# CG-Labs/HAN

Measured on AMD Instinct MI355X. Metric: full-graph train epochs/sec + node-attn HBM GB/s, 8-head HAN at 1/2/4/8 GPUs, higher is better.
Workload: dtype f32

## Files before the change

### han_amd/_lib.py

```python
from __future__ import annotations

import ctypes
import os
import subprocess
from ctypes import c_char_p, c_float, c_int, c_int64, c_size_t, c_uint64, c_void_p

_HERE = os.path.dirname(os.path.abspath(__file__))
LIB_PATH = os.path.join(_HERE, "libhan_hip.so")
CSRC = os.path.join(_HERE, "csrc")
SOURCES = ("node_attn.hip", "project.hip", "project_sparse.hip", "sem_attn.hip", "loss_opt.hip", "metapath.hip", "evaluate.hip",
           "ego_block.hip")
EXTRA_FLAGS = {"node_attn.hip": ("-mllvm", "-amdgpu-mfma-vgpr-form")}

P = c_void_p
I64 = c_int64


class HanRowSplit(ctypes.Structure):
    _fields_ = [("split_deg", c_int64), ("n_long", c_int64), ("n_chunks", c_int64),
                ("long_rows", c_void_p), ("long_ptr", c_void_p), ("chunk_long", c_void_p),
                ("chunk_start", c_void_p), ("chunk_end", c_void_p), ("workspace", c_void_p),
                ("workspace_bytes", c_size_t), ("n_short", c_int64), ("n_mid", c_int64),
                ("short_rows", c_void_p), ("mid_rows", c_void_p)]

# ... 1 lines not shown
class HanDense(ctypes.Structure):
    _fields_ = [("bits", c_void_p), ("ld_words", c_int64), ("n_table", c_int64), ("workspace", c_void_p),
                ("workspace_bytes", c_size_t)]


SIGNATURES = {
    "han_abi_version": (c_int, []),
    "han_error_string": (c_char_p, [c_int]),
    "han_project_fwd_workspace": (c_size_t, [I64, c_int, c_int, c_int]),
    "han_project_fwd_multi_workspace": (c_size_t, [I64, c_int, c_int, c_int, c_int]),
    "han_project_keep_bytes": (c_size_t, [I64, c_int, I64, c_int, c_int]),
    "han_project_fwd": (c_int, [P, c_int, I64, P, P, P, P, P, P, c_int, P, P, P, c_size_t, I64, c_int, c_int, c_int,
                                c_float, c_float, c_uint64, P, I64, P, c_int, P]),
    "han_project_fwd_multi": (c_int, [P, c_int, I64, P, P, P, P, P, P, c_int, P, P, P, c_size_t, I64, c_int, c_int, c_int,
                                      c_int, c_float, c_float, P, P, I64, P, c_int, P]),
    "han_project_bwd_workspace": (c_size_t, [I64, c_int, c_int, c_int]),
    "han_project_bwd": (c_int, [P, c_int, I64, P, P, P, c_size_t, I64, c_int, c_int, c_int, c_float,
                                c_uint64, P, I64, P, P]),
    "han_project_bwd_input": (c_int, [P, P, P, I64, I64, c_int, c_int, c_int, c_float, c_uint64, P, I64, P]),
    "han_project_sparse_fwd": (c_int, [P, P, P, P, P, P, P, P, P, c_int, P, P, I64, c_int, c_int, c_int, c_float, c_float,
                                       c_uint64, P, I64, c_int, P]),
    "han_project_sparse_bwd_workspace": (c_size_t, [I64]),
    "han_project_sparse_bwd": (c_int, [P, P, P, I64, I64, I64, P, P, P, P, P, P, P, P, c_size_t, I64, c_int, c_int, c_int,
                                       c_float, c_uint64, P, I64, P]),
    "han_row_split_workspace": (c_size_t, [I64]),
    "han_node_attn_fwd": (c_int, [P, P, P, P, c_int, P, P, P, P, P, P, P, P, I64, P, P, P, P, I64, I64, c_int,
                                  c_int, c_float, c_float, c_float, c_uint64, P, I64, c_int, c_int, P, P, P]),
    "han_node_attn_dense_workspace": (c_size_t, [I64, I64, c_int]),
    "han_csr_to_bitmask": (c_int, [P, P, I64, I64, P, I64, P, P]),
    "han_node_attn_coefs": (c_int, [P, P, P, P, P, P, P, c_int, I64, I64, c_int, c_int, c_float, c_float,
# ... 46 lines not shown
    "han_knn_topk": (c_int, [P, I64, P, I64, P, P, P, c_size_t, I64, I64, c_int, c_int, P]),
    "han_knn_vote": (c_int, [P, P, P, I64, c_int, I64, P]),
    "han_contingency": (c_int, [P, P, I64, c_int, c_int, P, P]),
    "han_kmeans_step_workspace": (c_size_t, [I64, c_int, c_int]),
    "han_kmeans_step": (c_int, [P, I64, P, P, P, P, P, P, P, P, P, c_size_t, I64, c_int, c_int, P]),
    "han_silhouette_workspace": (c_size_t, [I64, c_int, c_int]),
    "han_silhouette": (c_int, [P, I64, P, I64, c_int, c_int, P, P, P, P, P, c_size_t, P]),
    "han_tsne_workspace": (c_size_t, [I64, c_int]),
    "han_tsne_calibrate": (c_int, [P, I64, I64, c_int, c_float, c_float, c_int, c_int, P, P, P, P, P, P, c_size_t, P]),
    "han_tsne_step": (c_int, [P, I64, P, P, P, P, P, P, P, P, I64, c_int, c_float, c_float, c_float, c_float, c_int, P,
                              c_size_t, P]),
}

ABI_VERSION = 15
E_UNSUPPORTED = -2
_lib = None


class HanLibraryError(RuntimeError):
    pass


def build(force: bool = False, verbose: bool = False) -> str:
    from concurrent.futures import ThreadPoolExecutor
    hdrs = [os.path.join(CSRC, f) for f in os.listdir(CSRC) if f.endswith(".h")] + \
        [os.path.join(_HERE, "..", "include", "han_hip.h")]
    hdr_time = max(os.path.getmtime(h) for h in hdrs)
    objdir = os.path.join(CSRC, "build")
    os.makedirs(objdir, exist_ok=True)
    jobs, objs = [], []
# ... 59 lines not shown
```

### han_amd/csrc/loss_opt.hip

```cpp
#include "han_common.h"

namespace {

constexpr int MAXC = 16;
constexpr int kClsBlocks = 2048;

struct ClsArgs {
    const float *Z, *Wc, *bc;
    const int32_t *labels;
    const uint8_t *mask;
    float row_weight;
    float *logits, *dZ, *slab;
    int64_t N;
    int C, HC;
};

__device__ __forceinline__ float cls_row16_sum(float v) {
    v += han_dpp_xor16<1>(v);
    v += han_dpp_xor16<2>(v);
    v += han_dpp_xor16<4>(v);
    v += han_dpp_xor16<8>(v);
    return v;
}

// ... 462 lines not shown
    if (!bias || !rowptr || !colidx || N < 0 || ld < N) return HAN_E_BADARG;
    if (N == 0) return 0;
    bias_fill_kernel<<<(unsigned)((N + 3) / 4), 256, 0, (hipStream_t)stream>>>(bias, N, ld, rowptr, colidx);
    HAN_CHECK_LAUNCH();
    return 0;
}

extern "C" int han_abi_version(void) { return HAN_ABI_VERSION; }

extern "C" const char *han_error_string(int code) {
    switch (code) {
        case 0: return "ok";
        case HAN_E_BADARG: return "han: bad argument (null pointer, negative size or inconsistent shape)";
        case HAN_E_UNSUPPORTED: return "han: shape not supported by this build (K*FP == 64 with FP in {4,8,16,32,64}; D and A multiples of 64)";
        case HAN_E_WORKSPACE: return "han: workspace too small";
        default: return code > 0 ? hipGetErrorString((hipError_t)code) : "han: unknown error";
    }
}
```

### han_amd/csrc/project.hip

```cpp
#include "han_b6.h"
#include "han_k1_epilogue.h"

namespace {

constexpr int BM = 64;
constexpr int BK = 32;
constexpr int XS_LD = 34;
constexpr int WS_LD = 80;

struct ProjFwdArgs : K1Epilogue {
    const unsigned char *wimg;
    const void *X;
    int64_t ldx;
    const float *W;
    int x_bf16, F;
    uint32_t thr_in;
    float inv_keep_in;
    int f_chunk;
    float *partial;
    uint8_t *keep;
};

__device__ __forceinline__ float load_x1(const void *X, int bf, int64_t idx) {
    if (bf) return __uint_as_float((uint32_t)reinterpret_cast<const uint16_t *>(X)[idx] << 16);
// ... 340 lines not shown
#pragma unroll
    for (int m = 0; m < MT; ++m) {
#pragma unroll
        for (int r = 0; r < 4; ++r) {
            const int64_t row = row0 + 16 * (w * MT + m) + l4 * 4 + r;
            float vst[4];
#pragma unroll
            for (int t = 0; t < 4; ++t) {
                float v = acc[m][t][0][r];
                if (HPT > 1) v = myhh ? acc[m][t][HPT - 1][r] : v;
                if (DROP) v *= a.inv_keep_in;
                vst[t] = k1_store_elem(a, row, t, l15, v);
            }
            if (DROP && a.f1) tile_scores<8>(a, row, row < a.N, vst, a1c, a2c, l15);
        }
    }
}

struct ProjMultiArgs {
    const void *X;
    int64_t ldx;
    const float *W;
    const unsigned char *wimg;
    void *H;
    int h_bf16;
    int64_t N;
    int F;
    int p_first;
    int P;
    const float *a1, *a2, *b1, *b2;
// ... 722 lines not shown
        for (int p = 0; p < done && !m.fuse_scores; ++p) {
            rc = launch_scores(path_of(all, p, N, F, K, hb, kb), N, FP, h_bf16, st);
            if (rc != 0) return rc;
        }
    }
    for (int p = done; p < P; ++p) {
        const K1Path q = path_of(all, p, N, F, K, hb, kb);
        const int rc = han_project_fwd(X, x_dtype, ldx, q.W, q.a1, q.a2, q.b1, q.b2, q.H, table_dtype, q.f1, q.f2,
                                       workspace, workspace_bytes, N, F, K, FP, in_drop, fts_drop,
                                       seeds ? seeds[p] : 0, seed_dev, row_offset, q.keep, flags, stream);
        if (rc != 0) return rc;
    }
    return 0;
}

extern "C" size_t han_project_bwd_workspace(int64_t N, int F, int, int) {
    int ftiles; int64_t rpc, nch;
    bwd_geometry(N, F, &ftiles, &rpc, &nch);
    return (size_t)nch * (size_t)F * HAN_D * sizeof(float);
}

extern "C" int han_project_bwd(const void *X, int x_dtype, int64_t ldx, const float *dH, float *dW, void *workspace,
                               size_t workspace_bytes, int64_t N, int F, int K, int FP, float in_drop,
                               uint64_t seed, const uint64_t *seed_dev, int64_t row_offset, const uint8_t *keep,
                               void *stream) {
    if (!X || !dH || !dW || !workspace || N < 0 || F <= 0 || ldx < F) return HAN_E_BADARG;
    if (!han_fp_supported(K, FP)) return HAN_E_UNSUPPORTED;
    if (!han_k1_dtype(x_dtype)) return HAN_E_UNSUPPORTED;
    if (in_drop < 0.f || in_drop >= 1.f) return HAN_E_BADARG;
    if (workspace_bytes < han_project_bwd_workspace(N, F, K, FP)) return HAN_E_WORKSPACE;
// ... 44 lines not shown
```

### han_amd/gat.py

```python
from __future__ import annotations

import functools
import math

import torch
import torch.nn.functional as F_torch

from . import layers, ops, rng
from .base_gattn import BaseGAttN
from .dist import NodePartition
from .graph import CSRGraph, as_graph

D = ops.D


class _ClassOrInstance:

    def __init__(self, fn):
        self.fn = fn
        functools.update_wrapper(self, fn)

    def __get__(self, obj, objtype=None):
        if obj is None:
            obj = objtype.default_instance()
# ... 39 lines not shown
        torch.nn.Module.__init__(self)
        self._built = False
        self._device = torch.device(device) if device is not None else None
        self.partition: NodePartition | None = None
        self.halo_plans = (None, None)
        self.masked_bwd = None
        self.zero_rows = False
        self.live_bwd = None
        self.path_streams = None
        self.path_order = "index"
        self.overlap_branch = None
        self.fold_k3 = False
        self._fold_handover = None
        self._live_handover = None
        self.side_stream = None
        self._graph_cache: dict = {}
        self.step_seed_dev: torch.Tensor | None = None
        self._fixed_seeds: dict = {}

    @classmethod
    def default_instance(cls):
        if cls._default is None:
            cls._default = cls()
        return cls._default

    @classmethod
    def reset_default(cls):
        cls._default = None

    def build(self, n_metapaths, ft_size, nb_classes, hid_units=(8,), n_heads=(8, 1),
# ... 67 lines not shown
        if new_flat.dtype != torch.float32:
            raise TypeError("han_amd parameters are float32 (the kernels read fp32 parameters); "
                            "bf16 storage is selected with build(table_dtype=torch.bfloat16)")
        new_grad = fn(self.flat_grad)
        self._buffers["flat"], self._buffers["flat_grad"] = new_flat, new_grad
        off = 0
        for name, shp in self.param_shapes():
            n = math.prod(shp)
            v = self._views[name]
            v.data = new_flat[off:off + n].view(shp)
            v.grad = new_grad[off:off + n].view(shp)
            off += n
        self._graph_cache.clear()
        return self

    def param_shapes(self):
        return _param_shapes(self.P, self.F, self.K, self.FP, self.A, self.C, self.HC, self.extra,
                             self.residual)

    def direct_grads(self, flag: bool = True):
        for v in self._views.values():
            v._han_direct_grad = bool(flag)
        return self

    def zero_grad_flat(self):
        self.flat_grad.zero_()
        self._rebind_grads()

    def _rebind_grads(self):
        off = 0
# ... 39 lines not shown
            key = (layer, P)
            if key not in self._fixed_seeds:
                self._fixed_seeds[key] = tuple(rng.next_seed() for _ in graphs)
            return self._fixed_seeds[key]

        def run(layer, sd, **kw):
            first = layer == 0
            return layers.LayerRun(
                train=train, in_drop=float(ffd_drop), coef_drop=float(attn_drop), seeds=sd,
                seed_dev=self.step_seed_dev if train else None, act=act_code, part=self.partition, graphs_t=graphs_t,
                layer=layer, table_dtype=self.table_dtype, plans_f=self.halo_plans[0], plans_b=self.halo_plans[1],
                xs_full=xs_full if first else None, masked_bwd=self.masked_bwd if (first and train) else None,
                zero_rows=bool(self.zero_rows and first and train and not self.extra),
                live_bwd=self.live_bwd if (first and train and not self.extra and self.masked_bwd is None) else None,
                streams=self.path_streams, side_stream=self.side_stream, path_order=self.path_order,
                overlap=self.overlap_branch if (first and train) else None, **kw)

        def layer_fwd(layer, Xin, xs_, K, FP, sink):
            sfx = "" if layer == 0 else f"_{layer}"
            g = lambda n: getattr(self, n + sfx, None)
            W, a1, b1, a2, b2, c, Wr, br = (g(n) for n in ("W", "a1", "b1", "a2", "b2", "c", "Wr", "br"))
            sd = seeds(layer)
            wide = FP > GROUP
            groups = [(k, k + 1) for k in range(K)] if wide else _head_groups(K, FP)
            if fold is not None:
                fold.clear()
            if len(groups) == 1 and K * FP == GROUP:
                return layers.NodeLevelAttention.apply(Xin, W, a1, b1, a2, b2, c, Wr, br, xs_, tuple(graphs),
                                                       run(layer, sd, coef_sink=sink, coef_mean=True, fold_sink=fold,
                                                           live_fwd=live_fwd, live_sink=live_used))
            fn = layers.WideHeadAttention if wide else layers.NodeLevelAttention
# ... 136 lines not shown
```

### han_amd/layers.py

```python
from __future__ import annotations

import dataclasses
import functools
from typing import NamedTuple

import torch
import torch.nn.functional as F_torch

from . import ops, rng
from .dist import NodePartition
from .features import SparseFeatures, as_features, is_sparse_input
from .graph import as_graph

D = ops.D


def _act_code(activation):
    if activation is None:
        return ops.ACT_IDENTITY, None
    if activation in (F_torch.elu, torch.nn.functional.elu, "elu") or \
            isinstance(activation, torch.nn.ELU):
        return ops.ACT_ELU, None
    if activation == "identity":
        return ops.ACT_IDENTITY, None
# ... 73 lines not shown

    def __init__(self, graph):
        self.graph = graph

    def exchange(self, table, tag):
        return _Ready(table)


class AllGatherTable(LocalTable):

    def __init__(self, part: NodePartition, graph):
        self.part, self.graph = part, graph

    def exchange(self, table, tag):
        return self.part.all_gather_rows_async(table, tag)


@dataclasses.dataclass(frozen=True, eq=False)
class LayerRun:
    train: bool
    seeds: tuple
    act: int
    in_drop: float = 0.0
    coef_drop: float = 0.0
    seed_dev: torch.Tensor | None = None
    part: NodePartition | None = None
    graphs_t: tuple | None = None
    layer: int = 0
    group: int = 0
    table_dtype: torch.dtype = torch.float32
    plans_f: list | None = None
    plans_b: list | None = None
    xs_full: tuple | None = None
    masked_bwd: list | None = None
    zero_rows: bool = False
    streams: list | None = None
    side_stream: torch.cuda.Stream | None = None
    path_order: str | None = None
    overlap: object = None
    coef_sink: list | None = None
    coef_mean: bool = False
    fold_sink: list | None = None
    live_bwd: object = None
    live_fwd: object = None
    live_sink: list | None = None

    @functools.cached_property
    def multi(self) -> bool:
        return self.part is not None and self.part.active

    @functools.cached_property
    def row_offset(self) -> int:
        return self.part.row_start if self.part is not None else 0

    @functools.cached_property
    def drop_in(self) -> float:
        return float(self.in_drop) if self.train else 0.0

    @functools.cached_property
    def drop_coef(self) -> float:
# ... 157 lines not shown
        saved = [None] * P
        srcs = [run.source_f(p, graphs[p]) for p in range(P)]
        proj = [None] * P
        xs_full = run.xs_full if (multi and Xin is None) else None
        replicated = [xs_full is not None and isinstance(s, AllGatherTable) for s in srcs]
        pj = [None] * P
        shared = xs_full if all(replicated) else (xs if not any(replicated) else None)
        streams = run.streams if (not multi and run.streams is not None and len(run.streams) >= P) else None
        side = run.side_stream if (streams is None and not multi and train and P > 1 and W.is_cuda) else None
        _fork(streams)
        overlap = run.overlap if (train and run.group == 0) else None
        if overlap is not None:
            overlap.node_level()
        if streams is None and P > 1 and shared is not None and _same_tensor(shared) and W.is_contiguous() and _unit_stride(shared[0]):
            full = all(replicated)
            Hs, f1s, f2s, keeps = ops.project_fwd_multi(shared[0], W, a1, a2, b1, b2, in_drop=in_drop, fts_drop=in_drop,
                                                        seeds=[int(v) for v in run.seeds],
                                                        row_offset=0 if full else row_offset, table_dtype=tdt,
                                                        seed_dev=seed_dev, want_keep=True)
            pj = [(Hs[p], f1s[p], f2s[p], keeps[p]) for p in range(P)]

        def project_path(p):
            seed = int(run.seeds[p])
            X, off = (xs_full[p], 0) if replicated[p] else (xs[p], row_offset)
            H, f1, f2, keep = pj[p] if pj[p] is not None else ops.project_fwd(
                X, W[p], a1[p], a2[p], b1[p], b2[p], in_drop=in_drop, fts_drop=in_drop, seed=seed,
                row_offset=off, table_dtype=tdt, seed_dev=seed_dev, want_keep=True)
            if replicated[p]:
                handle, r0, r1 = _Ready(H), part.row_start, part.row_end
                H, f1, f2 = H[r0:r1], f1[r0:r1], f2[r0:r1]
                if keep is not None:
                    Fw = X.shape[1]
                    kb_loc = ops.keep_bytes(r1 - r0, Fw, xs[p].stride(0), K, FP)
                    keep = keep[r0 * Fw:r0 * Fw + kb_loc] if kb_loc and (r0 * Fw) % 8 == 0 else None
# ... 502 lines not shown
```

### han_amd/ops.py

```python
from __future__ import annotations

import contextlib
import ctypes

import torch

from . import _lib, csr
from .features import SparseFeatures
from .graph import CSRGraph

ACT_IDENTITY = 0
ACT_ELU = 1
FLAG_XCD_ORDER = 1
FLAG_LEAN = 256
FLAG_K2_DEEP = 512
K2_DEEP = False
K2_SHARED_HASH = False
K2_FULL_GATHER = False
FLAG_K2_FULL_GATHER = 2048
FLAG_K2_ZERO_ROWS = 4096
GS_Z_ALL_ZERO = 0x3F800000
FLAG_K2_ROW_SUBSET = 8192
FLAG_MASKED_EDGES = 64
FLAG_K1_EXACT_PIPE = 2
# ... 356 lines not shown
    xcode, ldx, N, F, K, FP, in_drop, fts_drop, H, f1, f2, ws, keep = _project_fwd_setup(
        X, W, a1, a2, b1, b2, (P,), in_drop, fts_drop, table_dtype, flags, want_keep,
        lib.han_project_fwd_multi_workspace)
    if (in_drop > 0 or fts_drop > 0) and (seeds is None or len(seeds) != P):
        raise ValueError("dropout needs one seed per meta-path")
    seed_arr = (ctypes.c_uint64 * P)(*[int(x) & ((1 << 64) - 1) for x in (seeds if seeds is not None else [0] * P)])
    _lib.check(lib.han_project_fwd_multi(
        X.data_ptr(), xcode, ldx, W.data_ptr(), a1.data_ptr(), a2.data_ptr(), b1.data_ptr(), b2.data_ptr(),
        H.data_ptr(), DTYPE_CODE[table_dtype], f1.data_ptr(), f2.data_ptr(),
        _ptr(ws), ws.numel() if ws is not None else 0, N, F, K, FP, P,
        in_drop, fts_drop, seed_arr, _dev_word(seed_dev), int(row_offset),
        _ptr(keep), int(flags), _stream()), "han_project_fwd_multi")
    if want_keep:
        return H, f1, f2, [keep[p] if keep is not None else None for p in range(P)]
    return H, f1, f2


def project_bwd(X, dH, K, FP, in_drop=0.0, seed=0, row_offset=0, seed_dev=None, out=None, keep=None):
    lib = _lib.load()
    if isinstance(X, SparseFeatures):
        if keep is not None:
            raise ValueError("keep: sparse features have no keep table")
        return _project_sparse_bwd(X, dH, K, FP, in_drop, seed, row_offset, seed_dev, out)
    _chk(X, "X", contiguous=False, dtype=X.dtype)
    xcode = _dtype_code(X, "X")
    N, F = X.shape
    _chk(dH, "dH", (N, D), device=X.device)
    _check_heads(K, FP)
    dW = _out(out, "out", (F, D), X.device)
    nbytes = lib.han_project_bwd_workspace(N, F, K, FP)
# ... 805 lines not shown
```

### han_amd/rng.py

```python
from __future__ import annotations

_state = {"seed": 0x243F6A8885A308D3, "counter": 0}
_MASK = (1 << 64) - 1


def manual_seed(seed: int) -> None:
    _state["seed"] = int(seed) & _MASK
    _state["counter"] = 0


def _splitmix64(x: int) -> int:
    x = (x + 0x9E3779B97F4A7C15) & _MASK
    z = x
    z = ((z ^ (z >> 30)) * 0xBF58476D1CE4E5B9) & _MASK
    z = ((z ^ (z >> 27)) * 0x94D049BB133111EB) & _MASK
    return z ^ (z >> 31)


def next_seed() -> int:
    _state["counter"] += 1
    return _splitmix64(_state["seed"] ^ _splitmix64(_state["counter"]))
```

### han_amd/trainer.py

```python
from __future__ import annotations

import os

import torch

from . import layers, ops, rng
from .base_gattn import TFAdam
from .dist import NodePartition
from .features import SparseFeatures, as_features
from .gat import HeteGAT_multi
from .graph import as_graph


class _EvalBranch:

    def __init__(self, trainer, stream):
        self.tr, self.stream = trainer, stream
        self.M = self.vl = self.va = None

    def _run(self, fn):
        m = self.tr.model
        streams, m.path_streams = m.path_streams, None
        branch, m.overlap_branch = getattr(m, "overlap_branch", None), None
        try:
# ... 25 lines not shown
            self.M = None
        self._run(fn)


LIVE_BACKWARD_MIN_ROWS = 262144


LIVE_FORWARD_MIN_ROWS = 262144


class HANTrainer:
    def __init__(self, model: HeteGAT_multi, xs, graphs, labels, train_mask, val_mask=None,
                 lr=0.005, l2_coef=0.001, attn_drop=0.6, ffd_drop=0.6,
                 part: NodePartition | None = None, patience=100, max_halo_fraction=0.6,
                 use_graph=False, graphs_local=False, xs_full=None, replicate="auto", masked_backward=False,
                 side_stream=False, overlap_eval=False, live_backward="auto", live_forward="auto"):
        if not model._built:
            raise RuntimeError("build the model first (model.build(...))")
        self.model = model
        model.direct_grads(True)
        model.fold_k3 = True
        self.part = part if (part is not None and part.active) else None
        layers._no_sparse_under_partition(self.part is not None or xs_full is not None, xs, xs_full)
        model.partition = self.part
        dev = model.flat.device
        self.xs_full, self.replicate, self.replicate_info = None, frozenset(), None
        self._replicate_arg = replicate
        if xs_full is not None and self.part is not None:
            from .dist import replication_policy
            pt = self.part
            if any(x.shape[0] != pt.n_global for x in xs_full):
# ... 54 lines not shown
        if live_forward is True and not fwd_ok(self.val_mask):
            raise ValueError("live_forward=True needs a CUDA model with one node-attention layer of 8 x 8 heads, at most "
                             "64 classes, no node partition and a val mask of at most half of the rows")
        if live_forward is True or (live_forward == "auto" and n_all >= LIVE_FORWARD_MIN_ROWS):
            if fwd_ok(self.val_mask):
                self._live_fwd[id(self.val_mask)] = (self.val_mask, layers.LiveForwardPlan(self.graphs, self.val_mask))
            A, P = model.w_omega.shape[1], len(self.graphs)
            if (self._live_plan is not None and shape_ok and A in (64, 128) and P in (1, 2, 4)
                    and tuple(model.w_omega.shape) == (ops.D, A) and n_all * ops.gs_row_bytes() < (1 << 32)):
                mine = self._live_fwd.get(id(self.train_mask))
                plan = layers.LiveForwardPlan(self.graphs, self.train_mask, backward=self._live_plan)
                if mine is not None:
                    plan._subsets = mine[1]._subsets
                self._live_fwd_train = plan

        self.w_train = 1.0 / max(self._global_count(self.train_mask), 1)
        self.w_val = 1.0 / max(self._global_count(self.val_mask), 1)
        n_global = self._global_count(torch.ones_like(self.train_mask))
        model.zero_rows = dev.type == "cuda" and not model.extra and 2 * self._global_count(self.train_mask) <= n_global
        self.opt = TFAdam(model.flat, model.flat_grad, lr=lr, l2_coef=l2_coef)
        self._one = torch.ones((), dtype=torch.float32, device=dev)
        self.attn_drop, self.ffd_drop = attn_drop, ffd_drop
        self.patience = patience
        self.vlss_mn, self.vacc_mx, self.curr_step = float("inf"), 0.0, 0
        self.best_state = None
        self.use_graph = bool(use_graph)
        if overlap_eval not in (False, True, "branch", "sections"):
            raise ValueError(f"overlap_eval = {overlap_eval!r}: expected False, True, 'branch' or 'sections'")
        self.overlap_eval = bool(overlap_eval)
        self.overlap_form = "sections" if overlap_eval == "sections" else "branch"
# ... 19 lines not shown
            model.step_seed_dev = self.step_state[0:1]
            self.opt.step_dev = self.step_state[1:2]
            if dev.type == "cuda" and os.environ.get("HAN_PATH_STREAMS", "1") != "0" and len(self.graphs) > 1:
                model.path_streams = [torch.cuda.Stream(device=dev) for _ in self.graphs]
            if self.overlap_eval:
                model.path_order = "heavy"
                self._flat_prev = torch.empty_like(model.flat)
                if dev.type == "cuda":
                    self._eval_stream = torch.cuda.Stream(device=dev)

    @property
    def live_backward(self) -> bool:
        return self.model.live_bwd is not None

    @property
    def live_forward(self) -> bool:
        return id(self.val_mask) in self._live_fwd

    def set_masked_backward(self, flag: bool):
        self.masked_backward = bool(flag)
        self.model.live_bwd = None if self.masked_backward else self._live_plan
        if not self.masked_backward:
            self.model.masked_bwd = None
            return
        if getattr(self, "use_graph", False) and self._graph is not None:
            raise RuntimeError("the epoch is already captured; choose masked_backward before the first epoch")
        if self.model.extra:
            raise NotImplementedError("masked_backward needs a single node-attention layer: with more, the rows "
                                      "outside the mask feed the rows inside it")
        if self._masked_plans is None:
# ... 83 lines not shown
        if self.part is not None:
            self.part.all_reduce_sum_(self.model.flat_grad)
        self.opt.step()
        return loss.detach(), acc

    def eval_step(self, mask=None, weight=None):
        mask = self.val_mask if mask is None else mask
        weight = self.w_val if weight is None else weight
        loss, acc = self._forward(False, mask, weight)
        return loss, acc

    def epoch(self):
        if self.use_graph:
            return self._epoch_graph()
        tl, ta = self.train_step()
        vl, va = self.eval_step()
        return tl, ta, vl, va

    def _epoch_body(self):
        self.step_state.add_(self._step_inc)
        if self.overlap_eval:
            return self._epoch_body_overlapped()
        tl, ta = self.train_step()
        vl, va = self.eval_step()
        return tl, ta, vl, va

    def _eval_branch(self):
        br = _EvalBranch(self, None)
        br.node_level()
        br.head()
        return br.vl, br.va
# ... 86 lines not shown
              "signature": self._signature(),
              "rng": dict(rng._state),
              "fixed_seeds": {f"{k[0]}:{k[1]}": list(v) for k, v in self.model._fixed_seeds.items()},
              "step_state": self.step_state.cpu() if self.use_graph else None,
              "early_stop": {"vlss_mn": self.vlss_mn, "vacc_mx": self.vacc_mx, "curr_step": self.curr_step},
              "best_state": self.best_state.cpu() if self.best_state is not None else None}
        torch.save(ck, path)

    def load_checkpoint(self, path):
        ck = torch.load(path, weights_only=True)
        sig = self._signature()
        if ck.get("signature") != sig:
            raise ValueError("checkpoint was written for a different model / trainer configuration: "
                             f"{ck.get('signature')} vs {sig}")
        m = self.model
        m.flat.copy_(ck["flat"])
        self.opt.load_state_dict(ck["opt"])
        rng._state.update(ck["rng"])
        fixed = {(int(k.split(":")[0]), int(k.split(":")[1])): tuple(v) for k, v in ck["fixed_seeds"].items()}
        if self._graph is not None and fixed != m._fixed_seeds:
            raise RuntimeError("this trainer has already captured its epoch with other per-meta-path seed "
                               "constants baked in; load the checkpoint before the first epoch")
        m._fixed_seeds = fixed
        if self.use_graph:
            self.step_state.copy_(ck["step_state"])
            self.step_state[1] = self.opt.t
        es = ck["early_stop"]
        self.vlss_mn, self.vacc_mx, self.curr_step = float(es["vlss_mn"]), float(es["vacc_mx"]), int(es["curr_step"])
        self.best_state = ck["best_state"].to(m.flat.device) if ck["best_state"] is not None else None

    def restore_best(self):
        if self.best_state is not None:
            self.model.flat.copy_(self.best_state)
```

### include/han_hip.h

```cpp
#ifndef HAN_HIP_H
#define HAN_HIP_H

#include <stddef.h>
#include <stdint.h>

#ifdef __cplusplus
extern "C" {
#endif

#define HAN_ABI_VERSION 15

#define HAN_E_BADARG   (-1)
#define HAN_E_UNSUPPORTED (-2)
#define HAN_E_WORKSPACE (-3)

#define HAN_ACT_IDENTITY 0
#define HAN_ACT_ELU      1
#define HAN_FLAG_XCD_ORDER 1

#define HAN_FLAG_LEAN 256
#define HAN_FLAG_K2_DEEP 512
#define HAN_FLAG_K2_SHARED_HASH 1024
#define HAN_FLAG_K2_FULL_GATHER 2048
#define HAN_FLAG_K2_ZERO_ROWS 4096
#define HAN_FLAG_MASKED_EDGES 64
#define HAN_FLAG_K2_ROW_SUBSET 8192
#define HAN_FLAG_K1_EXACT_PIPE  2
#define HAN_FLAG_K1_MATRIX_PIPE 4
#define HAN_FLAG_K1_PAIRS      32
// ... 16 lines not shown
size_t han_project_keep_bytes(int64_t N, int F, int64_t ldx, int K, int FP);
int han_project_fwd(const void *X, int x_dtype, int64_t ldx, const float *W, const float *a1,
                    const float *a2, const float *b1, const float *b2, void *H,
                    int table_dtype, float *f1, float *f2, void *workspace,
                    size_t workspace_bytes, int64_t N, int F, int K, int FP,
                    float in_drop, float fts_drop, uint64_t seed, const uint64_t *seed_dev, int64_t row_offset,
                    uint8_t *keep, int flags, void *stream);

int han_project_fwd_multi(const void *X, int x_dtype, int64_t ldx, const float *W, const float *a1,
                          const float *a2, const float *b1, const float *b2, void *H, int table_dtype,
                          float *f1, float *f2, void *workspace, size_t workspace_bytes, int64_t N,
                          int F, int K, int FP, int P, float in_drop, float fts_drop,
                          const uint64_t *seeds, const uint64_t *seed_dev, int64_t row_offset,
                          uint8_t *keep, int flags, void *stream);

size_t han_project_bwd_workspace(int64_t N, int F, int K, int FP);
int han_project_bwd(const void *X, int x_dtype, int64_t ldx, const float *dH, float *dW,
                    void *workspace, size_t workspace_bytes, int64_t N, int F, int K,
                    int FP, float in_drop, uint64_t seed, const uint64_t *seed_dev, int64_t row_offset,
                    const uint8_t *keep, void *stream);

int han_project_bwd_input(const float *dH, const float *W, float *dX, int64_t ldo, int64_t N,
                          int F, int K, int FP, float in_drop, uint64_t seed, const uint64_t *seed_dev,
                          int64_t row_offset, void *stream);

int han_project_sparse_fwd(const int64_t *rowptr, const int32_t *colidx, const float *vals, const float *W,
                           const float *a1, const float *a2, const float *b1, const float *b2, void *H,
                           int table_dtype, float *f1, float *f2, int64_t N, int F, int K, int FP,
                           float in_drop, float fts_drop, uint64_t seed, const uint64_t *seed_dev,
                           int64_t row_offset, int flags, void *stream);
// ... 219 lines not shown
```

Before: 100.1.

## Fuse eval and next-step dropout projection into one kernel and stash train tables

Adds a combined HIP kernel that computes, in one pass over X, both the no-dropout eval projection and the dropout-masked train projection for the next step, using peeked RNG seeds. The train tables are stashed and reused by the following train step when the step counter, parameter version, seeds, input and row offset all match. This is meant to remove the second full read of the feature matrix and the separate train projection launch each epoch. In exchange it holds extra device memory for the stashed tables and adds invalidation logic on checkpoint load and best-state restore. It is only enabled for a narrow configuration: unpartitioned, 8x8 heads, fp32, an even number of meta-paths and enough free memory.

```diff
diff --git a/han_amd/_lib.py b/han_amd/_lib.py
--- a/han_amd/_lib.py
+++ b/han_amd/_lib.py
@@ -39,6 +39,9 @@
                                 c_float, c_float, c_uint64, P, I64, P, c_int, P]),
     "han_project_fwd_multi": (c_int, [P, c_int, I64, P, P, P, P, P, P, c_int, P, P, P, c_size_t, I64, c_int, c_int, c_int,
                                       c_int, c_float, c_float, P, P, I64, P, c_int, P]),
+    "han_project_fwd_both_workspace": (c_size_t, [I64, c_int, c_int, c_int, c_int]),
+    "han_project_fwd_both": (c_int, [P, c_int, I64, P, P, P, P, P, P, c_int, P, P, P, P, P, P, c_size_t, I64, c_int, c_int,
+                                     c_int, c_int, c_float, c_float, P, P, I64, P, c_int, P]),
     "han_project_bwd_workspace": (c_size_t, [I64, c_int, c_int, c_int]),
     "han_project_bwd": (c_int, [P, c_int, I64, P, P, P, c_size_t, I64, c_int, c_int, c_int, c_float,
                                 c_uint64, P, I64, P, P]),
@@ -115,6 +118,7 @@
 
 ABI_VERSION = 15
 E_UNSUPPORTED = -2
+E_NOT_ELIGIBLE = -4
 _lib = None
 
 
diff --git a/han_amd/csrc/loss_opt.hip b/han_amd/csrc/loss_opt.hip
--- a/han_amd/csrc/loss_opt.hip
+++ b/han_amd/csrc/loss_opt.hip
@@ -500,6 +500,7 @@
         case HAN_E_BADARG: return "han: bad argument (null pointer, negative size or inconsistent shape)";
         case HAN_E_UNSUPPORTED: return "han: shape not supported by this build (K*FP == 64 with FP in {4,8,16,32,64}; D and A multiples of 64)";
         case HAN_E_WORKSPACE: return "han: workspace too small";
+        case HAN_E_NOT_ELIGIBLE: return "han: this call is outside the combined kernel's shapes; nothing was launched (use the separate entry points)";
         default: return code > 0 ? hipGetErrorString((hipError_t)code) : "han: unknown error";
     }
 }
diff --git a/han_amd/csrc/project.hip b/han_amd/csrc/project.hip
--- a/han_amd/csrc/project.hip
+++ b/han_amd/csrc/project.hip
@@ -378,6 +378,166 @@
             }
             if (DROP && a.f1) tile_scores<8>(a, row, row < a.N, vst, a1c, a2c, l15);
         }
+    }
+}
+
+struct ProjBothArgs {
+    ProjFwdArgs tr;
+    K1Epilogue ev;
+    int64_t wstep;
+};
+
+__global__ __launch_bounds__(512, 4) void project_fwd_b6_both_kernel(const ProjBothArgs b_in) {
+    ProjFwdArgs a = b_in.tr;
+    han_resolve_seed(a.seed_lo, a.seed_hi, a.seed_dev);
+    constexpr int NT = 512;
+    constexpr int XV = 1024 / NT;
+    constexpr int WU = (B6_WTILE / 8) / NT;
+    constexpr int ZB = B6_WTILE;
+    __shared__ __attribute__((aligned(16))) unsigned char lds[3 * B6_XBYTES + B6_WTILE + ZB + B6_ROWS * 128];
+    unsigned char *Xs = lds;
+    unsigned char *Ws = lds + 3 * B6_XBYTES;
+    unsigned char *Kacc = Ws + B6_WTILE + ZB;
+    const int tid = threadIdx.x;
+    const int lane = tid & 63, w = tid >> 6;
+    const int l15 = lane & 15, l4 = lane >> 4;
+    const int64_t row0 = (int64_t)blockIdx.x * B6_ROWS;
+#pragma unroll
+    for (int i = 0; i < ZB / (8 * NT); ++i)
+        *reinterpret_cast<uint2 *>(Ws + B6_WTILE + 8 * (tid + NT * i)) = make_uint2(0u, 0u);
+    static_assert(ZB % (8 * NT) == 0, "the mirror is zeroed in whole 8-byte pieces per thread");
+    auto flush_keep = [&](int kbase) {
+#pragma unroll
+        for (int i = 0; i < 1024 / NT; ++i) {
+            const int c = tid + NT * i;
+            const int r = c >> 3, sg = c & 7;
+            const int64_t krow = row0 + r;
+            if (krow < a.N && kbase + 16 * sg < a.F) {
+                const uint4 raw = *reinterpret_cast<const uint4 *>(Kacc + r * 128 + 16 * (sg ^ ((r >> 1) & 7)));
+                const uint4 v = (r & 1) ? make_uint4(raw.z, raw.w, raw.x, raw.y) : raw;
+                uint8_t *dst = a.keep + krow * (int64_t)a.F + kbase + 16 * sg;
+                if (kbase + 16 * sg + 8 < a.F) *reinterpret_cast<uint4 *>(dst) = v;
+                else *reinterpret_cast<uint2 *>(dst) = make_uint2(v.x, v.y);
+            }
+        }
+    };
+
+    f32x4 acc[4], acc_e[4];
+#pragma unroll
+    for (int t = 0; t < 4; ++t) acc[t] = acc_e[t] = (f32x4){0.f, 0.f, 0.f, 0.f};
+
+    float4_t xr[XV];
+    uint2 wq[WU];
+    const int ktiles = (a.F + 31) >> 5;
+    auto load_tile = [&](int k0) {
+#pragma unroll
+        for (int i = 0; i < XV; ++i) {
+            const int idx = tid + NT * i;
+            const int r = idx >> 3, c4 = (idx & 7) * 4;
+            const int64_t row = row0 + r;
+            const int64_t rc = row < a.N ? row : a.N - 1;
+            const int kc = k0 + c4 < a.F ? k0 + c4 : a.F - 4;
+            xr[i] = load_x4(a.X, false, rc * a.ldx + kc);
+        }
+        const int kt = (k0 >> 5) < ktiles ? (k0 >> 5) : ktiles - 1;
+        const unsigned char *src = a.wimg + (int64_t)kt * b_in.wstep;
+#pragma unroll
+        for (int i = 0; i < WU; ++i) wq[i] = *reinterpret_cast<const uint2 *>(src + 8 * (tid + NT * i));
+    };
+    const uint32_t thr2 = (a.thr_in & 0xFFFFu) * 0x00010001u, one2 = 0x00010001u;
+    const int fro = l15 * B6_LDB + ((l4 ^ b6_swz(l15)) << 4);
+    const int frz0 = fro + (l15 < 8 ? 0 : ZB), frz1 = fro + (l15 < 8 ? ZB : 0);
+    load_tile(0);
+    for (int k0 = 0; k0 < a.F; k0 += 32) {
+        __syncthreads();
+        if (k0 > 0 && (k0 & 96) == 0) flush_keep(k0 - 128);
+#pragma unroll
+        for (int i = 0; i < XV; ++i) {
+            const int idx = tid + NT * i;
+            b6_stage_x4<false>(Xs, B6_XBYTES, idx, row0 + (idx >> 3) < a.N && k0 + (idx & 7) * 4 < a.F, xr[i]);
+        }
+#pragma unroll
+        for (int i = 0; i < WU; ++i) *reinterpret_cast<uint2 *>(Ws + 8 * (tid + NT * i)) = wq[i];
+        __syncthreads();
+        load_tile(k0 + 32);
+        auto bfrag = [&](int t, int s3, int off) {
+            return *reinterpret_cast<const i32x4 *>(Ws + s3 * B6_WBYTES + 16 * t * B6_LDB + off);
+        };
+        const int lr = 16 * w + l15;
+        i32x4 af[3];
+#pragma unroll
+        for (int s3 = 0; s3 < 3; ++s3)
+            af[s3] = *reinterpret_cast<const i32x4 *>(Xs + s3 * B6_XBYTES + 16 * w * B6_LDB + fro);
+        const uint32_t nglob = (uint32_t)(row0 + lr + a.row_offset);
+        uint32_t kw[2] = {0u, 0u};
+#pragma unroll
+        for (int c = 0; c < 2; ++c) {
+            uint32_t mk[8][2];
+#pragma unroll
+            for (int j = 0; j < 8; ++j) {
+                const uint32_t kglob = (uint32_t)(k0 + 8 * l4 + j);
+                const HanRand64 rn = han_rand64(a.seed_lo, a.seed_hi, HAN_STREAM_SEQ, nglob, kglob * 2u + (uint32_t)c);
+                mk[j][0] = b6_keep_masks(rn.x, thr2, one2);
+                mk[j][1] = b6_keep_masks(rn.y, thr2, one2);
+#pragma unroll
+                for (int wd = 0; wd < 2; ++wd)
+                    kw[j >> 2] |= mk[j][wd] & (0x00010001u << (4 * (2 * c + wd) + (j & 3)));
+            }
+#pragma unroll
+            for (int hq = 0; hq < 4; ++hq) {
+                const int head = 4 * c + hq;
+                const int t = head >> 1, hh = head & 1, wd = hq >> 1;
+                const uint32_t sel = (head & 1) ? 0x07060302u : 0x05040100u;
+                i32x4 am[3];
+#pragma unroll
+                for (int i = 0; i < 4; ++i) {
+                    const uint32_t pm = __builtin_amdgcn_perm(mk[2 * i + 1][wd], mk[2 * i][wd], sel);
+#pragma unroll
+                    for (int s3 = 0; s3 < 3; ++s3) am[s3][i] = af[s3][i] & (int)pm;
+                }
+                if (hh == 0) {
+                    const i32x4 b0 = bfrag(t, 0, fro), b1 = bfrag(t, 1, fro), b2 = bfrag(t, 2, fro);
+                    acc_e[t] = han_b6_chain_k1<false>(af, b0, b1, b2, acc_e[t]);
+                }
+                const int fz = hh ? frz1 : frz0;
+                const i32x4 z0 = bfrag(t, 0, fz), z1 = bfrag(t, 1, fz), z2 = bfrag(t, 2, fz);
+                acc[t] = han_b6_chain_k1<false>(am, z0, z1, z2, acc[t]);
+            }
+        }
+        *reinterpret_cast<uint2 *>(Kacc + lr * 128 + 8 * ((((k0 & 96) >> 3) + l4) ^ (lr & 15))) = make_uint2(kw[0], kw[1]);
+    }
+    __syncthreads();
+    flush_keep(((a.F - 1) >> 7) << 7);
+    float a1c[4], a2c[4];
+    k1_tile_coeffs(a, l15, a1c, a2c);
+#pragma unroll
+    for (int r = 0; r < 4; ++r) {
+        const int64_t row = row0 + 16 * w + l4 * 4 + r;
+        float vst[4];
+#pragma unroll
+        for (int t = 0; t < 4; ++t) vst[t] = k1_store_elem(a, row, t, l15, acc[t][r] * a.inv_keep_in);
+        tile_scores<8>(a, row, row < a.N, vst, a1c, a2c, l15);
+    }
+    const K1Epilogue &e = b_in.ev;
+    k1_tile_coeffs(e, l15, a1c, a2c);
+#pragma unroll
+    for (int r = 0; r < 4; ++r) {
+        const int64_t row = row0 + 16 * w + l4 * 4 + r;
+        float vst[4];
+#pragma unroll
+        for (int t = 0; t < 4; ++t) {
+            const float v = acc_e[t][r];
+            const int64_t o = row * HAN_D + 16 * t + l15;
+            if (e.h_bf16) {
+                const uint32_t b = han_f32_to_bf16_bits(v);
+                if (row < a.N) reinterpret_cast<uint16_t *>(e.H)[o] = (uint16_t)b;
+                vst[t] = __uint_as_float(b << 16);
+            } else {
+                if (row < a.N) reinterpret_cast<float *>(e.H)[o] = v;
+                vst[t] = v;
+            }
+        }
+        tile_scores<8>(e, row, row < a.N, vst, a1c, a2c, l15);
     }
 }
 
@@ -1130,6 +1290,51 @@
     return 0;
 }
 
+extern "C" size_t han_project_fwd_both_workspace(int64_t N, int F, int K, int FP, int P) {
+    return k1_plan(N, F, F, K, FP, P).fwd_bytes;
+}
+
+extern "C" int han_project_fwd_both(const void *X, int x_dtype, int64_t ldx, const float *W, const float *a1,
+                                    const float *a2, const float *b1, const float *b2, void *H, int table_dtype,
+                                    float *f1, float *f2, void *H_eval, float *f1_eval, float *f2_eval, void *workspace,
+                                    size_t workspace_bytes, int64_t N, int F, int K, int FP, int P, float in_drop,
+                                    float fts_drop, const uint64_t *seeds, const uint64_t *seed_dev, int64_t row_offset,
+                                    uint8_t *keep, int flags, void *stream) {
+    if (P <= 0 || (in_drop > 0.f && !seeds)) return HAN_E_BADARG;
+    if (N == 0) return 0;
+    const K1Path all = {W, a1, a2, b1, b2, H, f1, f2, keep};
+    const int bad = han_k1_check_fwd(X, all, N, F, ldx >= F && H_eval && f1_eval && f2_eval, true, K, FP, x_dtype,
+                                     table_dtype, in_drop, fts_drop);
+    if (bad != 0) return bad;
+    if ((flags & HAN_FLAG_K1_EXACT_PIPE) && (flags & HAN_FLAG_K1_MATRIX_PIPE)) return HAN_E_BADARG;
+    const K1Plan plan = k1_plan(N, F, ldx, K, FP, P);
+    const bool vec = x_vec(X, ldx, F, false);
+    const bool fp32 = x_dtype == HAN_DTYPE_F32 && table_dtype == HAN_DTYPE_F32;
+    if (!(fp32 && in_drop > 0.f && keep && plan.keep_table && P % 2 == 0 && !(flags & HAN_FLAG_K1_4WAVE) &&
+          use_b6(plan, vec, false, in_drop, K, FP, flags) && use_fused(plan, vec, P, 0.f, 0.f, flags)))
+        return HAN_E_NOT_ELIGIBLE;
+    hipStream_t st = (hipStream_t)stream;
+    const int rc = launch_wimage(W, workspace, workspace_bytes, F, P, st);
+    if (rc != 0) return rc;
+    const size_t hb = (size_t)N * HAN_D * sizeof(float), kb = (size_t)N * (size_t)F + 128;
+    const K1Path all_e = {W, a1, a2, b1, b2, H_eval, f1_eval, f2_eval, nullptr};
+    const dim3 grid((unsigned)((N + B6_ROWS - 1) / B6_ROWS));
+    for (int p = 0; p < P; ++p) {
+        const K1Path q = path_of(all, p, N, F, K, hb, kb);
+        ProjBothArgs b;
+        static_cast<K1Epilogue &>(b.tr) = han_k1_epilogue(q, true, table_dtype, N, seeds[p], seed_dev, fts_drop, flags, row_offset);
+        b.tr.X = X; b.tr.ldx = ldx; b.tr.W = q.W; b.tr.F = F; b.tr.x_bf16 = 0;
+        b.tr.thr_in = han_drop_threshold(in_drop); b.tr.inv_keep_in = 1.f / (1.f - in_drop);
+        b.tr.keep = q.keep; b.tr.f_chunk = plan.f_chunk; b.tr.partial = nullptr;
+        b.tr.wimg = (const unsigned char *)workspace + (size_t)p * B6_WTILE;
+        b.wstep = (int64_t)P * B6_WTILE;
+        b.ev = han_k1_epilogue(path_of(all_e, p, N, F, K, hb, 0), true, table_dtype, N, 0, nullptr, 0.f, 0, 0);
+        project_fwd_b6_both_kernel<<<grid, 512, 0, st>>>(b);
+        HAN_CHECK_LAUNCH();
+    }
+    return 0;
+}
+
 extern "C" size_t han_project_bwd_workspace(int64_t N, int F, int, int) {
     int ftiles; int64_t rpc, nch;
     bwd_geometry(N, F, &ftiles, &rpc, &nch);
diff --git a/han_amd/gat.py b/han_amd/gat.py
--- a/han_amd/gat.py
+++ b/han_amd/gat.py
@@ -77,6 +77,7 @@
         self._fold_handover = None
         self._live_handover = None
         self.side_stream = None
+        self.shared_proj = None
         self._graph_cache: dict = {}
         self.step_seed_dev: torch.Tensor | None = None
         self._fixed_seeds: dict = {}
@@ -174,6 +175,11 @@
         self._graph_cache.clear()
         return self
 
+    def load_state_dict(self, *args, **kw):
+        if self.shared_proj is not None:
+            self.shared_proj.drop()
+        return super().load_state_dict(*args, **kw)
+
     def param_shapes(self):
         return _param_shapes(self.P, self.F, self.K, self.FP, self.A, self.C, self.HC, self.extra,
                              self.residual)
@@ -243,7 +249,8 @@
                 zero_rows=bool(self.zero_rows and first and train and not self.extra),
                 live_bwd=self.live_bwd if (first and train and not self.extra and self.masked_bwd is None) else None,
                 streams=self.path_streams, side_stream=self.side_stream, path_order=self.path_order,
-                overlap=self.overlap_branch if (first and train) else None, **kw)
+                overlap=self.overlap_branch if (first and train) else None,
+                shared_proj=self.shared_proj if (first and not self.extra) else None, **kw)
 
         def layer_fwd(layer, Xin, xs_, K, FP, sink):
             sfx = "" if layer == 0 else f"_{layer}"
diff --git a/han_amd/layers.py b/han_amd/layers.py
--- a/han_amd/layers.py
+++ b/han_amd/layers.py
@@ -111,6 +111,51 @@
 
     def exchange(self, table, tag):
         return self.part.all_gather_rows_async(table, tag)
+
+
+def stash_key(step, flat):
+    return (int(step), int(flat._version), int(flat.data_ptr()))
+
+
+class SharedProjection:
+
+    def __init__(self, flat_of, step_of):
+        self._flat_of, self._step_of = flat_of, step_of
+        self.armed = None
+        self._stash = None
+        self.taken = 0
+
+    def key(self):
+        return stash_key(self._step_of(), self._flat_of())
+
+    @staticmethod
+    def stash_bytes(N, F, P):
+        return P * (N * D * 4 + 2 * N * 8 * 4 + N * F + 128)
+
+    def drop(self):
+        self._stash = None
+
+    def eval_forward(self, X, W, a1, a2, b1, b2, row_offset, tdt):
+        self._stash = None
+        P = W.shape[0]
+        seeds = rng.peek_seeds(P)
+        got = ops.project_fwd_both(X, W, a1, a2, b1, b2, self.armed, self.armed, seeds, row_offset=row_offset,
+                                   table_dtype=tdt)
+        if got is None:
+            return None
+        self._stash = (self.key(), X, float(self.armed), tuple(seeds), int(row_offset), tdt, got[0])
+        return got[1]
+
+    def take(self, X, in_drop, seeds, row_offset, tdt):
+        st, self._stash = self._stash, None
+        if st is None:
+            return None
+        key, Xs, drop, sds, off, tdt_s, tables = st
+        if (Xs is X and drop == float(in_drop) and sds == tuple(int(v) for v in seeds) and off == int(row_offset)
+                and tdt_s == tdt and key == self.key()):
+            self.taken += 1
+            return tables
+        return None
 
 
 @dataclasses.dataclass(frozen=True, eq=False)
@@ -141,6 +186,7 @@
     live_bwd: object = None
     live_fwd: object = None
     live_sink: list | None = None
+    shared_proj: object = None
 
     @functools.cached_property
     def multi(self) -> bool:
@@ -328,10 +374,16 @@
             overlap.node_level()
         if streams is None and P > 1 and shared is not None and _same_tensor(shared) and W.is_contiguous() and _unit_stride(shared[0]):
             full = all(replicated)
-            Hs, f1s, f2s, keeps = ops.project_fwd_multi(shared[0], W, a1, a2, b1, b2, in_drop=in_drop, fts_drop=in_drop,
-                                                        seeds=[int(v) for v in run.seeds],
-                                                        row_offset=0 if full else row_offset, table_dtype=tdt,
-                                                        seed_dev=seed_dev, want_keep=True)
+            off = 0 if full else row_offset
+            sp, got = run.shared_proj if seed_dev is None else None, None
+            if sp is not None and train:
+                got = sp.take(shared[0], in_drop, run.seeds, off, tdt)
+            elif sp is not None and sp.armed is not None:
+                ev = sp.eval_forward(shared[0], W, a1, a2, b1, b2, off, tdt)
+                got = ev + ([None] * P,) if ev is not None else None
+            Hs, f1s, f2s, keeps = got if got is not None else ops.project_fwd_multi(
+                shared[0], W, a1, a2, b1, b2, in_drop=in_drop, fts_drop=in_drop, seeds=[int(v) for v in run.seeds],
+                row_offset=off, table_dtype=tdt, seed_dev=seed_dev, want_keep=True)
             pj = [(Hs[p], f1s[p], f2s[p], keeps[p]) for p in range(P)]
 
         def project_path(p):
diff --git a/han_amd/ops.py b/han_amd/ops.py
--- a/han_amd/ops.py
+++ b/han_amd/ops.py
@@ -394,6 +394,29 @@
     if want_keep:
         return H, f1, f2, [keep[p] if keep is not None else None for p in range(P)]
     return H, f1, f2
+
+
+def project_fwd_both(X, W, a1, a2, b1, b2, in_drop, fts_drop, seeds, row_offset=0, table_dtype=torch.float32,
+                     seed_dev=None, flags=0):
+    lib = _lib.load()
+    if isinstance(X, SparseFeatures) or X.dim() != 2 or W.dim() != 3:
+        return None
+    P = a1.shape[0]
+    xcode, ldx, N, F, K, FP, in_drop, fts_drop, H, f1, f2, ws, keep = _project_fwd_setup(
+        X, W, a1, a2, b1, b2, (P,), in_drop, fts_drop, table_dtype, flags, True, lib.han_project_fwd_both_workspace)
+    if seeds is None or len(seeds) != P:
+        raise ValueError("one seed per meta-path")
+    He, f1e, f2e = torch.empty_like(H), torch.empty_like(f1), torch.empty_like(f2)
+    seed_arr = (ctypes.c_uint64 * P)(*[int(x) & ((1 << 64) - 1) for x in seeds])
+    code = lib.han_project_fwd_both(
+        X.data_ptr(), xcode, ldx, W.data_ptr(), a1.data_ptr(), a2.data_ptr(), b1.data_ptr(), b2.data_ptr(),
+        H.data_ptr(), DTYPE_CODE[table_dtype], f1.data_ptr(), f2.data_ptr(), He.data_ptr(), f1e.data_ptr(), f2e.data_ptr(),
+        _ptr(ws), ws.numel() if ws is not None else 0, N, F, K, FP, P, in_drop, fts_drop, seed_arr, _dev_word(seed_dev),
+        int(row_offset), _ptr(keep), int(flags), _stream())
+    if code == _lib.E_NOT_ELIGIBLE:
+        return None
+    _lib.check(code, "han_project_fwd_both")
+    return (H, f1, f2, [keep[p] for p in range(P)]), (He, f1e, f2e)
 
 
 def project_bwd(X, dH, K, FP, in_drop=0.0, seed=0, row_offset=0, seed_dev=None, out=None, keep=None):
diff --git a/han_amd/rng.py b/han_amd/rng.py
--- a/han_amd/rng.py
+++ b/han_amd/rng.py
@@ -20,3 +20,8 @@
 def next_seed() -> int:
     _state["counter"] += 1
     return _splitmix64(_state["seed"] ^ _splitmix64(_state["counter"]))
+
+
+def peek_seeds(n: int) -> tuple:
+    c = _state["counter"]
+    return tuple(_splitmix64(_state["seed"] ^ _splitmix64(c + i)) for i in range(1, int(n) + 1))
diff --git a/han_amd/trainer.py b/han_amd/trainer.py
--- a/han_amd/trainer.py
+++ b/han_amd/trainer.py
@@ -63,7 +63,8 @@
                  lr=0.005, l2_coef=0.001, attn_drop=0.6, ffd_drop=0.6,
                  part: NodePartition | None = None, patience=100, max_halo_fraction=0.6,
                  use_graph=False, graphs_local=False, xs_full=None, replicate="auto", masked_backward=False,
-                 side_stream=False, overlap_eval=False, live_backward="auto", live_forward="auto"):
+                 side_stream=False, overlap_eval=False, live_backward="auto", live_forward="auto",
+                 shared_projection="auto"):
         if not model._built:
             raise RuntimeError("build the model first (model.build(...))")
         self.model = model
@@ -148,6 +149,27 @@
                     plan._subsets = mine[1]._subsets
                 self._live_fwd_train = plan
 
+        if shared_projection not in ("auto", True, False):
+            raise ValueError(f"shared_projection = {shared_projection!r}: expected 'auto', True or False")
+        model.shared_proj = None
+        x0 = self.xs[0] if self.xs else None
+        P_ = len(self.graphs)
+        share_ok = (dev.type == "cuda" and not model.extra and self.part is None and not use_graph and not overlap_eval
+                    and model.K == 8 and model.FP == 8 and model.table_dtype == torch.float32 and P_ >= 2 and P_ % 2 == 0
+                    and float(ffd_drop) > 0 and isinstance(x0, torch.Tensor) and x0.dtype == torch.float32
+                    and all(x is x0 for x in self.xs)
+                    and ops.keep_bytes(x0.shape[0], x0.shape[1], x0.stride(0), 8, 8) > 0
+                    and bool(torch.isfinite(x0).all()))
+        if shared_projection is True and not share_ok:
+            raise ValueError("shared_projection=True needs a CUDA model with one node-attention layer of 8 x 8 heads and fp32 "
+                             "tables, one dense fp32 feature tensor of at least 32 768 rows shared by an even number of "
+                             "meta-paths, input dropout, no node partition, no captured epoch and no overlap_eval")
+        if share_ok and shared_projection == "auto":
+            need = layers.SharedProjection.stash_bytes(x0.shape[0], x0.shape[1], P_)
+            share_ok = 4 * need <= torch.cuda.mem_get_info(dev)[0]
+        if share_ok and shared_projection is not False:
+            model.shared_proj = layers.SharedProjection(lambda: model.flat, lambda: self.opt.t)
+
         self.w_train = 1.0 / max(self._global_count(self.train_mask), 1)
         self.w_val = 1.0 / max(self._global_count(self.val_mask), 1)
         n_global = self._global_count(torch.ones_like(self.train_mask))
@@ -197,6 +219,14 @@
         return self.model.live_bwd is not None
 
     @property
+    def shared_projection(self) -> bool:
+        return self.model.shared_proj is not None
+
+    def _drop_shared(self):
+        if self.model.shared_proj is not None:
+            self.model.shared_proj.drop()
+
+    @property
     def live_forward(self) -> bool:
         return id(self.val_mask) in self._live_fwd
 
@@ -310,7 +340,15 @@
         if self.use_graph:
             return self._epoch_graph()
         tl, ta = self.train_step()
-        vl, va = self.eval_step()
+        sp = self.model.shared_proj
+        if sp is None:
+            vl, va = self.eval_step()
+            return tl, ta, vl, va
+        sp.armed = float(self.ffd_drop)
+        try:
+            vl, va = self.eval_step()
+        finally:
+            sp.armed = None
         return tl, ta, vl, va
 
     def _epoch_body(self):
@@ -427,6 +465,7 @@
             raise ValueError("checkpoint was written for a different model / trainer configuration: "
                              f"{ck.get('signature')} vs {sig}")
         m = self.model
+        self._drop_shared()
         m.flat.copy_(ck["flat"])
         self.opt.load_state_dict(ck["opt"])
         rng._state.update(ck["rng"])
@@ -444,4 +483,5 @@
 
     def restore_best(self):
         if self.best_state is not None:
+            self._drop_shared()
             self.model.flat.copy_(self.best_state)
diff --git a/include/han_hip.h b/include/han_hip.h
--- a/include/han_hip.h
+++ b/include/han_hip.h
@@ -13,6 +13,7 @@
 #define HAN_E_BADARG   (-1)
 #define HAN_E_UNSUPPORTED (-2)
 #define HAN_E_WORKSPACE (-3)
+#define HAN_E_NOT_ELIGIBLE (-4)
 
 #define HAN_ACT_IDENTITY 0
 #define HAN_ACT_ELU      1
@@ -59,6 +60,14 @@
                           const uint64_t *seeds, const uint64_t *seed_dev, int64_t row_offset,
                           uint8_t *keep, int flags, void *stream);
 
+size_t han_project_fwd_both_workspace(int64_t N, int F, int K, int FP, int P);
+int han_project_fwd_both(const void *X, int x_dtype, int64_t ldx, const float *W, const float *a1,
+                         const float *a2, const float *b1, const float *b2, void *H, int table_dtype,
+                         float *f1, float *f2, void *H_eval, float *f1_eval, float *f2_eval, void *workspace,
+                         size_t workspace_bytes, int64_t N, int F, int K, int FP, int P, float in_drop,
+                         float fts_drop, const uint64_t *seeds, const uint64_t *seed_dev, int64_t row_offset,
+                         uint8_t *keep, int flags, void *stream);
+
 size_t han_project_bwd_workspace(int64_t N, int F, int K, int FP);
 int han_project_bwd(const void *X, int x_dtype, int64_t ldx, const float *dH, float *dW,
                     void *workspace, size_t workspace_bytes, int64_t N, int F, int K,
```

After: 102.8, median of 6. +2.7%, better.
